# LayoutLLM-T2I/LayoutLLM-T2I

Measured on AMD Instinct MI355X. Metric: 512x512 50-step images/sec (PLMS, CFG 7.5, layout-conditioned GLIGEN UNet), higher is better.
Workload: dtype fp16 (fp32 accumulate); 1 GPU; configs[1]: 512x512, 50 PLMS steps, batch=4/GPU, 8 grounding boxes/image, fp16; survey_config=2, unet_forwards_per_image=102, parallelism=replicas x1, one weight broadcast, no per-step collectives

## Files before the change

layoutllm_t2i_amd/csrc/gemm_conv.hip:

```cpp
#include <atomic>
#include <cstring>
#include "common.h"
#include "gligen_hip.h"
#include "gemm_shared.h"
#include "opts.h"

namespace {

#define g_opt_ksplit gl_opt(13)
#define g_opt_geglu32 gl_opt(8)
#define g_opt_big gl_opt(7)
#define g_opt_small gl_opt(4)
#define g_opt_splitk_tiles gl_opt(5)
#define g_opt_splitk_tiles_conv gl_opt(GL_OPT_SPLITK_TILES_CONV)
#define g_opt_splitk_nk gl_opt(6)
#define g_opt_skinny gl_opt(24)
#define g_opt_order gl_opt(23)
#define g_opt_tile gl_opt(2)
#define g_opt_g8 gl_opt(30)
#define g_opt_g8_tiles gl_opt(31)
#define g_opt_g8_tapmajor gl_opt(33)
#define g_opt_g8_minkt gl_opt(34)
std::atomic<uint64_t> g8_launches{0};
#define g_opt_g8_shortk gl_opt(37)
#define g_opt_g8_bm128 gl_opt(46)
#define g_opt_g8_minblk gl_opt(47)
#define g_opt_g8_s3 gl_opt(52)
#define g_opt_g8_minnk gl_opt(35)

template <int BM, int BN, int BKT, int NW = 4>
constexpr int lds_bytes() {
    constexpr int pipe = 2 * (BM + BN) * BKT * (int)sizeof(half_t);
    constexpr int epi = NW * 32 * 68 * (int)sizeof(float);
    return pipe > epi ? pipe : epi;
}

template <int BM, int BN, int BKT, int WK = 1>
constexpr int min_waves() {
    if (WK > 1) return 2;
    if (BKT != 32) return 1;
    if (BM * BN >= 256 * 128) return 2;
    if (BM * BN <= 128 * 128) return 4;
    return 3;
}

template <int BM, int BN, int WAVES_M, int WAVES_N, bool CONV, int BKT, int WK = 1>
__global__ __launch_bounds__(64 * WAVES_M * WAVES_N * WK, (min_waves<BM, BN, BKT, WK>())) void gemm_kernel(gl_gemm_args p, ConvGeom cg, int splitk, int kt_per_split, int order_m) {
    constexpr int NTHR = 64 * WAVES_M * WAVES_N * WK;
    constexpr int TM = BM / WAVES_M / 32;
    constexpr int TN = BN / WAVES_N / 32;
    constexpr int CPR = BKT / 8;
    constexpr int RPP = NTHR / CPR;
    constexpr int RPW = 64 / CPR;
    constexpr int APASS = (BM + RPP - 1) / RPP;
    constexpr int BPASS = (BN + RPP - 1) / RPP;
    constexpr int KSTEPS = BKT / 16;
    static_assert(WAVES_M * WAVES_N * WK == 4, "4 waves");
    static_assert(WK == 1 || (WK == 2 && TM == 2 && KSTEPS % 2 == 0), "K-split: two groups, two 32-row tiles per wave");
    static_assert(BM % RPW == 0 && BN % RPW == 0, "whole wave instructions");
    static_assert(BKT == 64 || BKT == 32, "BK");

    extern __shared__ __attribute__((aligned(16))) unsigned char smem[];
    half_t* As = reinterpret_cast<half_t*>(smem);
    half_t* Bs = As + 2 * BM * BKT;

    const int tid = threadIdx.x;
    const int lane = tid & 63;
    const int wave = tid >> 6;
    const int wk = wave / (WAVES_M * WAVES_N);
    const int wmn = wave - wk * (WAVES_M * WAVES_N);
    const int wm = wmn / WAVES_N;
    const int wn = wmn % WAVES_N;
    const int M = p.M, N = p.N, K = p.K;
    const int nt = (N + BN - 1) / BN;
    int tile;
    {
        const int nwg = gridDim.x;
        const int bid = blockIdx.x;
        const int q = nwg >> 3, r = nwg & 7;
        const int xcd = bid & 7, local = bid >> 3;
        tile = (xcd < r ? xcd * (q + 1) : r * (q + 1) + (xcd - r) * q) + local;
    }
    const int mt_ = (M + BM - 1) / BM;
    const int tm = order_m ? tile % mt_ : tile / nt;
    const int m0 = tm * BM;
    const int n0 = (order_m ? tile / mt_ : tile - tm * nt) * BN;
    const int kt_begin = blockIdx.z * kt_per_split;
    const int kt_end = min(K / BKT, kt_begin + kt_per_split);
    const int nkt = kt_end - kt_begin;

    const int srow = tid / CPR;
    const int skc = tid % CPR;
    auto swz = [](int r) -> int { return BKT == 64 ? ((r >> 1) & 7) : ((r >> 2) & 3); };

    const half_t* __restrict__ Ag = reinterpret_cast<const half_t*>(p.a);
    const half_t* __restrict__ A2g = reinterpret_cast<const half_t*>(p.a2);
    const half_t* __restrict__ Wg = reinterpret_cast<const half_t*>(p.w);
    const half_t* zsrc = reinterpret_cast<const half_t*>(g_zero16);

// ... 328 lines not shown
                    const int pc = (lane & 3) * 8;
                    const int m = mbase + r;
                    const int nx = nbase + pc;
                    if (m < M && nx < N) {
                        const float4 x0 = *reinterpret_cast<const float4*>(stage + r * EPS + pc);
                        const float4 x1 = *reinterpret_cast<const float4*>(stage + r * EPS + pc + 4);
                        const float4 g0 = *reinterpret_cast<const float4*>(stage + r * EPS + pc + 32);
                        const float4 g1 = *reinterpret_cast<const float4*>(stage + r * EPS + pc + 36);
                        float xv[8] = {x0.x, x0.y, x0.z, x0.w, x1.x, x1.y, x1.z, x1.w};
                        float gv[8] = {g0.x, g0.y, g0.z, g0.w, g1.x, g1.y, g1.z, g1.w};
                        half8_t o, lo8 = {};
#pragma unroll
                        for (int j = 0; j < 8; ++j) {
                            float a = xv[j], b = gv[j];
                            if (bias) { a += bias[nx + j]; b += bias[nx + 32 + j]; }
                            float y = a * gelu_erf_f(b);
                            if (p.out_mode == GL_OUT_F16_HILO) y = pin_value(y);
                            o[j] = (half_t)y;
                            if (p.out_mode == GL_OUT_F16_HILO) lo8[j] = (half_t)(y - (float)o[j]);
                        }
                        st16(outp + (size_t)m * p.ldc + (nbase >> 1) + pc, *reinterpret_cast<uint4*>(&o));
                        if (p.out_mode == GL_OUT_F16_HILO) st16(outp + (size_t)m * p.ldc + (N >> 1) + (nbase >> 1) + pc, *reinterpret_cast<uint4*>(&lo8));
                    }
                }
            } else {
                const int ncols = (np * 2 + 1 < TN) ? 64 : 32;
#pragma unroll
                for (int ps = 0; ps < 4; ++ps) {
                    const int r = ps * 8 + (lane >> 3);
                    const int c = (lane & 7) * 8;
                    const int m = mbase + r;
                    const int n = nbase + c;
                    if (c < ncols && m < M && n < N) {
                        const float4 a0 = *reinterpret_cast<const float4*>(stage + r * EPS + c);
                        const float4 a1 = *reinterpret_cast<const float4*>(stage + r * EPS + c + 4);
                        float v[8] = {a0.x, a0.y, a0.z, a0.w, a1.x, a1.y, a1.z, a1.w};
                        finish8(p, gate, m, n, v);
                    }
                }
            }
        }
    }
}

__global__ __launch_bounds__(256) void splitk_reduce_kernel(gl_gemm_args p, int splitk) {
    const int M = p.M, N = p.N;
    const int nq = N / 8;
    const size_t total = (size_t)M * nq;
    const float* ws = reinterpret_cast<const float*>(p.workspace);
    float gate = 1.0f;
    if (p.epi == GL_EPI_GATE_RES) gate = p.gate[0];
    const size_t zstride = (size_t)M * N;
    for (unsigned idx = blockIdx.x * 256u + threadIdx.x; idx < (unsigned)total; idx += gridDim.x * 256u) {
        const int m = (int)(idx / (unsigned)nq);
        const int n = (int)(idx - (unsigned)m * (unsigned)nq) * 8;
        const float* src = ws + (size_t)m * N + n;
        float4 a = *reinterpret_cast<const float4*>(src);
        float4 c = *reinterpret_cast<const float4*>(src + 4);
        int z = 1;
        for (; z + 1 < splitk; z += 2) {
            const float4 b0 = *reinterpret_cast<const float4*>(src + (size_t)z * zstride);
            const float4 d0 = *reinterpret_cast<const float4*>(src + (size_t)z * zstride + 4);
            const float4 b1 = *reinterpret_cast<const float4*>(src + (size_t)(z + 1) * zstride);
            const float4 d1 = *reinterpret_cast<const float4*>(src + (size_t)(z + 1) * zstride + 4);
            a.x += b0.x; a.y += b0.y; a.z += b0.z; a.w += b0.w;
            c.x += d0.x; c.y += d0.y; c.z += d0.z; c.w += d0.w;
            a.x += b1.x; a.y += b1.y; a.z += b1.z; a.w += b1.w;
            c.x += d1.x; c.y += d1.y; c.z += d1.z; c.w += d1.w;
        }
        for (; z < splitk; ++z) {
            const float4 b = *reinterpret_cast<const float4*>(src + (size_t)z * zstride);
            const float4 d = *reinterpret_cast<const float4*>(src + (size_t)z * zstride + 4);
            a.x += b.x; a.y += b.y; a.z += b.z; a.w += b.w;
            c.x += d.x; c.y += d.y; c.z += d.z; c.w += d.w;
        }
        float v[8] = {a.x, a.y, a.z, a.w, c.x, c.y, c.z, c.w};
        finish8(p, gate, m, n, v);
    }
}

constexpr int SK_BATCH = 20;
constexpr int SK_RS = 36;

__global__ __launch_bounds__(256) void gemm_skinny_kernel(gl_gemm_args p) {
    __shared__ __attribute__((aligned(16))) float part[4][32 * SK_RS];
    const int lane = threadIdx.x & 63, wave = threadIdx.x >> 6;
    const int n0 = blockIdx.x * 32, m0 = blockIdx.y * 32;
    const int M = p.M, K = p.K;
    const int steps = K / 64;
    const int kw = wave * steps * 16;
    int mr = m0 + (lane & 31);
    if (mr >= M) mr = M - 1;
    const half_t* ap = reinterpret_cast<const half_t*>(p.a) + (size_t)mr * p.lda + kw + 8 * (lane >> 5);
    const half_t* wp = reinterpret_cast<const half_t*>(p.w) + (size_t)(n0 + (lane & 31)) * p.ldw + (p.kwrap != 0 && kw >= p.kwrap ? kw - p.kwrap : kw) +
                       8 * (lane >> 5);
    f32x16 acc;
#pragma unroll
    for (int j = 0; j < 16; ++j) acc[j] = 0.0f;
    for (int s0 = 0; s0 < steps; s0 += SK_BATCH) {
        uint4 af[SK_BATCH], wf[SK_BATCH];
#pragma unroll
        for (int j = 0; j < SK_BATCH; ++j)
            if (s0 + j < steps) {
                af[j] = ld16(ap + (s0 + j) * 16);
                wf[j] = ld16(wp + (s0 + j) * 16);
            }
#pragma unroll
        for (int j = 0; j < SK_BATCH; ++j)
            if (s0 + j < steps)
                acc = __builtin_amdgcn_mfma_f32_32x32x16_f16(*reinterpret_cast<half8_t*>(&wf[j]), *reinterpret_cast<half8_t*>(&af[j]), acc, 0, 0, 0);
    }
    float* mine = part[wave] + (lane & 31) * SK_RS + 4 * (lane >> 5);
#pragma unroll
    for (int rg = 0; rg < 4; ++rg)
        *reinterpret_cast<float4*>(mine + 8 * rg) = make_float4(acc[rg * 4], acc[rg * 4 + 1], acc[rg * 4 + 2], acc[rg * 4 + 3]);
    __syncthreads();
    if (threadIdx.x < 128) {
        const int r = threadIdx.x >> 2, c = (threadIdx.x & 3) * 8;
        const int m = m0 + r;
        if (m < M) {
            float v[8];
#pragma unroll
            for (int j = 0; j < 8; ++j) v[j] = part[0][r * SK_RS + c + j];
#pragma unroll
            for (int w = 1; w < 4; ++w)
#pragma unroll
                for (int j = 0; j < 8; ++j) v[j] += part[w][r * SK_RS + c + j];
            float gate = 1.0f;
            if (p.epi == GL_EPI_GATE_RES) gate = p.gate[0];
            finish8(p, gate, m, n0 + c, v);
        }
    }
}

inline bool skinny_ok(const gl_gemm_args& g) {
    if (!g_opt_skinny || g.M > 1024 || (g.N % 32) != 0 || g.epi == GL_EPI_GEGLU || g.vt != nullptr || g.a2 != nullptr) return false;
    if (g.kwrap != 0 && g.K != 2 * g.kwrap) return false;
    if (g.out_mode == GL_OUT_F32_NCHW || (g.lda % 8) != 0) return false;
    if (g.K > 4096 && g.workspace != nullptr) return false;
    const long tiles = (long)gl_cdiv(g.M, 32) * (g.N / 32);
    return tiles * 64L * g.K * 2L <= (long)g_opt_skinny << 20;
}

inline int choose_splitk(const gl_gemm_args& g, int tiles, bool conv) {
    const int nk = g.K / 64;
    if (!g.workspace || g.epi == GL_EPI_GEGLU || g.out_mode == GL_OUT_F32_NCHW || g.vt != nullptr) return 1;
    if (tiles >= (conv ? g_opt_splitk_tiles_conv : g_opt_splitk_tiles) || nk < g_opt_splitk_nk) return 1;
    int s = (480 + tiles - 1) / tiles;
    if (s > nk / 8) s = nk / 8;
    if (s > 16) s = 16;
    while (s > 1 && (int64_t)s * g.M * g.N * 4 > g.workspace_bytes) --s;
    return s < 2 ? 1 : s;
}

template <int BM, int BN, int WM, int WN, bool CONV, int BKT, int WK = 1>
int launch(const gl_gemm_args& g, const ConvGeom& cg, hipStream_t st) {
    if (g.a2 != nullptr && (g.ksplit % BKT) != 0) return GL_ERR_BAD_ARG;
    if (g.vt != nullptr && ((g.vt_col0 % BN) % 64) != 0) return GL_ERR_UNSUPPORTED;
    const int mt = gl_cdiv(g.M, BM), nt = gl_cdiv(g.N, BN);
    const int nk = g.K / BKT;
    int splitk = choose_splitk(g, mt * nt, CONV);
    int kper = gl_cdiv(nk, splitk);
    const int zs = gl_cdiv(nk, kper);
    dim3 grid(mt * nt, 1, zs);
    constexpr int lds = lds_bytes<BM, BN, BKT, WM * WN * WK>();
    const int order_m = g_opt_order == 1 ? ((CONV ? 9L : 1L) * g.N > (long)g.M) : (g_opt_order == 2);
    gemm_kernel<BM, BN, WM, WN, CONV, BKT, WK><<<grid, dim3(64 * WM * WN * WK), lds, st>>>(g, cg, zs, kper, order_m);
    GL_CHECK_LAUNCH();
    if (zs > 1) {
        const size_t total = (size_t)g.M * (g.N / 8);
        int nblk = (int)((total + 255) / 256);
        if (nblk > 2048) nblk = 2048;
        splitk_reduce_kernel<<<dim3(nblk), dim3(256), 0, st>>>(g, zs);
        GL_CHECK_LAUNCH();
    }
    return 0;
}

template <bool CONV, int BKT>
int dispatch_shape(const gl_gemm_args& g, const ConvGeom& cg, hipStream_t st) {
    const bool geglu = (g.epi == GL_EPI_GEGLU);
    const bool rowmajor = (g.out_mode != GL_OUT_F32_NCHW);
    int shape = 0;
    if (g.N < 256 && (g.N % 128) != 0) shape = 2;
    else if (!geglu && (g.N % 160) == 0 && ((g.N % 128) != 0 || CONV || g_opt_tile == 2)) shape = 1;
    if (g_opt_tile == 1 && g.N >= 256) shape = 0;
    if (g_opt_small && !CONV && g.K <= 1280 && shape != 2 && (g.N % 128) == 0) {
        const long t128 = (long)gl_cdiv(g.M, 128) * gl_cdiv(g.N, shape == 1 ? 160 : 128);
        if (t128 < g_opt_small) shape = 3;
    }
    if constexpr (BKT == 64) {
        if (g_opt_ksplit && rowmajor && (shape == 0 || shape == 1)) {
            const int nk = g.K / 64;
            bool use = (g_opt_ksplit == 2);
            if (g_opt_ksplit == 1 || g_opt_ksplit == 3 || g_opt_ksplit == 4) use = CONV ? (shape == 1 && nk >= 20) : (nk >= 16);
            if (g_opt_ksplit == 3 && !CONV) use = false;
            if (g_opt_ksplit == 4 && CONV) use = false;
            if (use) {
                if (shape == 1) return launch<128, 160, 2, 1, CONV, 64, 2>(g, cg, st);
                return launch<128, 128, 2, 1, CONV, 64, 2>(g, cg, st);
            }
        }
        if (g_opt_big && shape != 2 && shape != 3 && g.M >= 256 && !(shape == 1 && g.vt != nullptr)) {
            const int bn = (shape == 1) ? 160 : 128;
            const long t256 = (long)gl_cdiv(g.M, 256) * gl_cdiv(g.N, bn);
            if (t256 >= g_opt_big) {
                if (shape == 1) return launch<256, 160, 4, 1, CONV, 32>(g, cg, st);
                return launch<256, 128, 4, 1, CONV, 32>(g, cg, st);
            }
        }
        if constexpr (!CONV) {
            if (shape == 3 && (g_opt_ksplit == 2 || ((g_opt_ksplit == 1 || g_opt_ksplit == 4 || g_opt_ksplit == 5) && g.K >= 1024)))
                return launch<64, 128, 1, 2, false, 64, 2>(g, cg, st);
        }
        if (shape == 3) return launch<64, 128, 2, 2, CONV, 64>(g, cg, st);
        if (shape == 1) return launch<128, 160, 4, 1, CONV, 64>(g, cg, st);
        if (shape == 0) return launch<128, 128, 2, 2, CONV, 64>(g, cg, st);
        return launch<256, 64, 4, 1, CONV, 64>(g, cg, st);
    } else {
        static_assert(!CONV, "BK 32 dispatch is for plain GEMMs");
        if (shape == 3) return launch<64, 128, 2, 2, false, 32>(g, cg, st);
        return launch<128, 128, 2, 2, false, 32>(g, cg, st);
    }
}

template <bool CONV>
int dispatch(const gl_gemm_args& g, const ConvGeom& cg, hipStream_t st) {
    if (g.M <= 0 || g.N <= 0 || g.K <= 0 || (g.K % 64) != 0) return GL_ERR_BAD_ARG;
    if (g.out_mode < 0 || g.out_mode > GL_OUT_F16_HILO) return GL_ERR_BAD_ARG;
    if (g.out_mode == GL_OUT_F16_HILO && g.ldc < (g.epi == GL_EPI_GEGLU ? g.N : 2 * g.N)) return GL_ERR_BAD_ARG;
    if ((g.vt != nullptr && (g.out_mode == GL_OUT_F16_HILO) != (g.vt_lo != nullptr)) || (g.vt == nullptr && g.vt_lo != nullptr)) return GL_ERR_BAD_ARG;
    if (g.out_mode != GL_OUT_F32_NCHW && ((g.N % 8) != 0 || (g.ldc % 8) != 0)) return GL_ERR_BAD_ARG;
    if (g.out_mode == GL_OUT_F32_ROWMAJOR && g.out2 != nullptr && (g.ldc2 % 8) != 0) return GL_ERR_BAD_ARG;
    if (g.out_mode == GL_OUT_F32_ROWMAJOR && g.epi == GL_EPI_GEGLU) return GL_ERR_UNSUPPORTED;
    if (g.res != nullptr && (g.ldres % 8) != 0) return GL_ERR_BAD_ARG;
    if (g.rowbias != nullptr && (g.ld_rowbias % 8) != 0) return GL_ERR_BAD_ARG;
    if (g.epi == GL_EPI_GEGLU && (g.N % 64) != 0) return GL_ERR_BAD_ARG;
    if (g.a2 != nullptr && (g.ksplit % 64) != 0) return GL_ERR_BAD_ARG;
    if ((g.epi == GL_EPI_RES || g.epi == GL_EPI_GATE_RES) && g.res == nullptr) return GL_ERR_BAD_ARG;
    if (g.epi == GL_EPI_GATE_RES && g.gate == nullptr) return GL_ERR_BAD_ARG;
    if (g.epi == GL_EPI_ROWBIAS && (g.rowbias == nullptr || g.rows_per_sample <= 0)) return GL_ERR_BAD_ARG;
    if (g.vt != nullptr && (g.epi != GL_EPI_BIAS || (g.out_mode != GL_OUT_F16_ROWMAJOR && g.out_mode != GL_OUT_F16_HILO) || (g.vt_col0 % 64) != 0 || g.vt_col0 <= 0 ||
                            g.vt_col0 >= g.N || g.vt_rows <= 0 || g.vt_d <= 0 || ((g.N - g.vt_col0) % g.vt_d) != 0 || (g.vt_ld % 8) != 0 ||
                            g.vt_ld < g.vt_rows || g.vt_H * g.vt_d != g.N - g.vt_col0))
        return GL_ERR_BAD_ARG;
    if constexpr (!CONV) {
        if (g.vt_lo == nullptr && skinny_ok(g)) {
            gemm_skinny_kernel<<<dim3(g.N / 32, gl_cdiv(g.M, 32)), dim3(256), 0, st>>>(g);
            GL_CHECK_LAUNCH();
            return 0;
        }
    }
    const bool need8 = g.vt_lo != nullptr;
    if (need8) {
        int bn_ = 0;
        if (!g_opt_g8 || !gl8_supported(g, CONV, &bn_)) return GL_ERR_UNSUPPORTED;
    }
    const bool upf = CONV && cg.ups == 2;
    auto mtiles = [&](const int bm_) { return upf ? 4 * gl_cdiv(g.M / 4, bm_) : gl_cdiv(g.M, bm_); };
    if (g_opt_g8 || upf) {
        int bn = 0;
        if (gl8_supported(g, CONV, &bn, upf)) {
            const int nk = g.K / 64;
            auto plan_split = [&](const int tiles_) {
                int sk = 1;
                if (tiles_ < g_opt_g8_tiles && g.workspace && g.epi != GL_EPI_GEGLU && g.vt == nullptr) {
                    sk = 256 / tiles_;
                    if (sk > nk / g_opt_g8_minkt) sk = nk / g_opt_g8_minkt;
                    while (sk > 1 && (int64_t)sk * g.M * g.N * 4 > g.workspace_bytes) --sk;
                    if (sk < 1) sk = 1;
                }
                return sk;
            };
            int bm = 256;
            int tiles = mtiles(256) * gl_cdiv(g.N, bn);
            int splitk = plan_split(tiles);
            if (tiles * 2 <= 256 && g.epi != GL_EPI_GEGLU && g.vt == nullptr) {
                const bool want = CONV ? ((g_opt_g8_bm128 & 4) || ((g_opt_g8_bm128 & 1) && nk / splitk <= 16)) : ((g_opt_g8_bm128 & 2) != 0);
                if (want) {
                    bm = 128;
                    tiles = mtiles(128) * gl_cdiv(g.N, bn);
                    splitk = plan_split(tiles);
                }
            }
            if (!CONV && (g_opt_g8_bm128 & 8) && bm == 256 && splitk == 1 && tiles > 256 && g.epi != GL_EPI_GEGLU) {
                const int t128 = gl_cdiv(g.M, 128) * gl_cdiv(g.N, bn);
                auto fills = [](const int b) { return b * 5 >= ((b + 255) / 256) * 256 * 4; };
                if (!fills(tiles) && fills(t128) && t128 <= 2048) {
                    bm = 128;
                    tiles = t128;
                }
            }
            if (!CONV && splitk > 1 && nk / splitk < 20) splitk = nk / 20 > 0 ? nk / 20 : 1;
            bool enough = tiles * splitk >= (CONV ? g_opt_g8_tiles : (g_opt_g8_minblk < g_opt_g8_tiles ? g_opt_g8_minblk : g_opt_g8_tiles)) && nk >= g_opt_g8_minnk;
            if (!CONV && enough) {
                const int blocks = tiles * splitk;
                const bool full_rounds = g_opt_g8_shortk && blocks * 5 >= ((blocks + 255) / 256) * 256 * 4;
                enough = nk >= 16 || blocks <= 256 || (g.epi == GL_EPI_GEGLU && (nk >= 10 || full_rounds)) || (full_rounds && blocks <= 2048);
            }
            if (g_opt_g8 == 2 || enough || need8 || upf) {
                const bool s3 = g_opt_g8_s3 != 0 && g.kwrap != 0 && g.K == 3 * g.kwrap &&
                                (CONV ? cg.cwrap != 0 : (g.a2 == g.a && g.lda2 == g.lda && g.ksplit == 2 * g.kwrap));
                const int nks = s3 ? g.kwrap / 32 : nk;
                const int kper = gl_cdiv(nks, splitk);
                const int zs = gl_cdiv(nks, kper);
                const int order_m = g_opt_order == 1 ? ((CONV ? 9L : 1L) * g.N > (long)g.M) : (g_opt_order == 2);
                const int e = gl8_launch(g, cg, CONV, bm, bn, zs, kper, order_m | (CONV && g_opt_g8_tapmajor ? 2 : 0), st, s3);
                if (e) return e;
                if (!upf) g8_launches.fetch_add(1, std::memory_order_relaxed);
                if (zs > 1) {
                    const size_t total = (size_t)g.M * (g.N / 8);
                    int nblk = (int)((total + 255) / 256);
                    if (nblk > 2048) nblk = 2048;
                    splitk_reduce_kernel<<<dim3(nblk), dim3(256), 0, st>>>(g, zs);
                    GL_CHECK_LAUNCH();
                }
                return 0;
            }
        }
    }
    if (upf) return GL_ERR_UNSUPPORTED;
    if constexpr (!CONV) {
        if (g_opt_geglu32 && g.epi == GL_EPI_GEGLU && g.K <= 640 && g.a2 == nullptr) return dispatch_shape<false, 32>(g, cg, st);
    }
    return dispatch_shape<CONV, 64>(g, cg, st);
}

}

extern "C" int gl_gemm(const gl_gemm_args* a, void* stream) {
    if (!a || !a->a || !a->w || !a->out) return GL_ERR_BAD_ARG;
    ConvGeom cg{};
    gl_gemm_args g = *a;
    if (g.kwrap != 0 && ((g.kwrap % 64) != 0 || g.kwrap >= g.K || g.K > 3 * g.kwrap)) return GL_ERR_BAD_ARG;
    if (g.ldw == 0) g.ldw = g.kwrap != 0 ? g.kwrap : g.K;
    if (g.ldw < (g.kwrap != 0 ? (g.K > 2 * g.kwrap ? 2 * g.kwrap : g.kwrap) : g.K) || (g.ldw % 8) != 0) return GL_ERR_BAD_ARG;
    return dispatch<false>(g, cg, (hipStream_t)stream);
}

namespace {
int conv3x3_entry(const gl_conv_args* a, int shift, void* stream) {
    if (!a || !a->in || !a->g.w || !a->g.out) return GL_ERR_BAD_ARG;
    if ((a->Cin % 64) != 0) return GL_ERR_BAD_ARG;
    if (a->stride != 1 && a->stride != 2) return GL_ERR_BAD_ARG;
    if (a->upsample2x < 0 || a->upsample2x > 2) return GL_ERR_BAD_ARG;
    if (a->upsample2x && (a->stride != 1 || a->Hout != 2 * a->Hin || a->Wout != 2 * a->Win)) return GL_ERR_BAD_ARG;
    const bool upf = a->upsample2x == 2;
    if (upf && (shift != 0 || a->in_split != 0 || a->w_split != 0 || a->g.out_mode == GL_OUT_F32_NCHW || a->g.out_mode == GL_OUT_F16_HILO ||
                a->g.epi == GL_EPI_GEGLU || a->g.vt != nullptr || a->g.vt_lo != nullptr))
        return GL_ERR_BAD_ARG;
    if (a->B >= 2048 || a->Hout >= 1024 || a->Wout >= 1024) return GL_ERR_BAD_ARG;
    if (a->in_split != 0 && a->in_split != 2 && a->in_split != 3) return GL_ERR_BAD_ARG;
    if (a->in_split == 3 && !a->w_split) return GL_ERR_BAD_ARG;
    gl_gemm_args g = a->g;
    g.a = a->in;
    g.a2 = nullptr;
    g.M = a->B * a->Hout * a->Wout;
    g.K = 9 * a->Cin * (a->in_split ? a->in_split : 1);
    g.ldw = 9 * a->Cin * (a->w_split ? 2 : 1);
    g.kwrap = a->in_split ? 9 * a->Cin : 0;
    if (upf) g.K = g.ldw = 4 * a->Cin;
    ConvGeom cg{reinterpret_cast<const half_t*>(a->in), a->B, a->Hin, a->Win, a->Cin * (a->in_split ? 2 : 1), a->Hout, a->Wout, a->stride,
                a->upsample2x, nullptr, a->in_split == 3 ? 2 * (a->Cin >> 6) : 0, shift};
    return dispatch<true>(g, cg, (hipStream_t)stream);
}
}

extern "C" int gl_conv3x3(const gl_conv_args* a, void* stream) { return conv3x3_entry(a, 0, stream); }

extern "C" int gl_conv3x3_pad01(const gl_conv_args* a, void* stream) {
    if (!a || a->stride != 2 || a->upsample2x != 0 || a->in_split != 0) return GL_ERR_BAD_ARG;
    if (a->Hout != a->Hin / 2 || a->Wout != a->Win / 2 || a->Hout <= 0 || a->Wout <= 0) return GL_ERR_BAD_ARG;
    return conv3x3_entry(a, 1, stream);
}

template <int BM, int BN, int WM, int WN, bool CONV, int BKT, int WK = 1>
int set_lds_attr() {
    hipError_t e = hipFuncSetAttribute((const void*)gemm_kernel<BM, BN, WM, WN, CONV, BKT, WK>,
                                       hipFuncAttributeMaxDynamicSharedMemorySize, lds_bytes<BM, BN, BKT, WM * WN * WK>());
    return e == hipSuccess ? 0 : (int)e;
}
template <int BM, int BN, int WM, int WN, int BKT, int WK = 1>
int set_lds_attr2() {
    int e = set_lds_attr<BM, BN, WM, WN, false, BKT, WK>();
    return e ? e : set_lds_attr<BM, BN, WM, WN, true, BKT, WK>();
}

extern "C" int gl_init_gemm(void) {
    int e;
    if ((e = set_lds_attr2<64, 128, 2, 2, 64>())) return e;
    if ((e = set_lds_attr2<128, 128, 2, 2, 64>())) return e;
    if ((e = set_lds_attr2<128, 160, 4, 1, 64>())) return e;
    if ((e = set_lds_attr2<256, 64, 4, 1, 64>())) return e;
    if ((e = set_lds_attr2<128, 160, 2, 1, 64, 2>())) return e;
    if ((e = set_lds_attr2<128, 128, 2, 1, 64, 2>())) return e;
    if ((e = set_lds_attr<64, 128, 1, 2, false, 64, 2>())) return e;
    if ((e = set_lds_attr2<256, 160, 4, 1, 32>())) return e;
    if ((e = set_lds_attr2<256, 128, 4, 1, 32>())) return e;
    if ((e = set_lds_attr<64, 128, 2, 2, false, 32>())) return e;
    if ((e = set_lds_attr<128, 128, 2, 2, false, 32>())) return e;
    if ((e = gl8_init())) return e;
    return 0;
}

int gl_attn_read_launch_counts(void* dst, int64_t bytes);

extern "C" int gl_debug_read(int what, void* dst, int64_t bytes) {
    if (what == 8) return gl8_read_stamps(dst, bytes);
    if (what == 10) return gl_attn_read_launch_counts(dst, bytes);
    if (what == 9 || what == 11 || what == 12) {
        if (!dst || bytes < (int64_t)sizeof(uint64_t)) return GL_ERR_BAD_ARG;
        const uint64_t n = what == 9 ? g8_launches.load(std::memory_order_relaxed) : (what == 11 ? gl8_kxr_launch_count() : gl8_upf_launch_count());
        memcpy(dst, &n, sizeof n);
        return 0;
    }
    return GL_ERR_BAD_ARG;
}
```

layoutllm_t2i_amd/csrc/misc.hip:

```cpp
#include "common.h"
#include "gligen_hip.h"
#include "opts.h"

namespace {

template <typename OT>
__global__ __launch_bounds__(256) void posnet_input_kernel(const float* __restrict__ boxes, const float* __restrict__ masks,
                                                           const float* __restrict__ emb, const float* __restrict__ null_pos,
                                                           const float* __restrict__ null_xyxy, int in_dim, int num_freqs,
                                                           OT* __restrict__ out) {
    const int row = blockIdx.x;
    const float m = masks[row];
    const int pos_dim = num_freqs * 8;
    OT* o = out + (size_t)row * (in_dim + pos_dim);
    for (int c = threadIdx.x; c < in_dim; c += 256) {
        const float v = emb[(size_t)row * in_dim + c] * m + (1.0f - m) * null_pos[c];
        o[c] = (OT)v;
    }
    for (int c = threadIdx.x; c < pos_dim; c += 256) {
        const int j = c / 8;
        const int r = c - j * 8;
        const int coord = r & 3;
        const float freq = powf(100.0f, (float)j / (float)num_freqs);
        const float arg = freq * boxes[(size_t)row * 4 + coord];
// ... 506 lines not shown

extern "C" int gl_pack_latent(const float* x, int32_t B, int32_t C, int32_t hw, int32_t Cpad, int32_t reps, int32_t split, void* out,
                              void* stream) {
    if (!x || !out || B <= 0 || C <= 0 || hw <= 0 || Cpad < (split ? 3 * C : C) || reps <= 0) return GL_ERR_BAD_ARG;
    pack_latent_kernel<<<dim3(ew_blocks((size_t)reps * B * hw * Cpad)), dim3(256), 0, (hipStream_t)stream>>>(
        x, B, C, hw, Cpad, reps, split, reinterpret_cast<half_t*>(out));
    GL_CHECK_LAUNCH();
    return 0;
}

extern "C" int gl_pack_latent_extra(const float* x, const float* extra, int32_t B, int32_t Bs, int32_t C, int32_t Ce, int32_t hw, int32_t Cpad,
                                    int32_t reps, int32_t split, void* out, void* stream) {
    if (!x || !extra || !out || B <= 0 || C <= 0 || Ce <= 0 || hw <= 0 || reps <= 0 || (Bs != 1 && Bs != B)) return GL_ERR_BAD_ARG;
    if (Cpad < (split ? 3 : 1) * (C + Ce)) return GL_ERR_BAD_ARG;
    pack_latent_extra_kernel<<<dim3(ew_blocks((size_t)reps * B * hw * Cpad)), dim3(256), 0, (hipStream_t)stream>>>(
        x, extra, B, Bs, C, Ce, hw, Cpad, reps, split, reinterpret_cast<half_t*>(out));
    GL_CHECK_LAUNCH();
    return 0;
}

extern "C" int gl_latent_blend(float* x, const float* x0, const float* noise, const float* mask, float a, float s, int32_t B, int32_t C,
                               int32_t hw, int32_t x0_batch, int32_t mask_batch, void* stream) {
    if (!x || !x0 || !noise || !mask || B <= 0 || C <= 0 || hw <= 0) return GL_ERR_BAD_ARG;
    if ((x0_batch != 1 && x0_batch != B) || (mask_batch != 1 && mask_batch != B)) return GL_ERR_BAD_ARG;
    const size_t n = (size_t)B * C * hw;
    const bool vec = (hw % 4) == 0 && ((reinterpret_cast<uintptr_t>(x) | reinterpret_cast<uintptr_t>(x0) | reinterpret_cast<uintptr_t>(noise) |
                                        reinterpret_cast<uintptr_t>(mask)) % 16) == 0;
    if (vec)
        latent_blend_kernel<4><<<dim3(ew_blocks(n / 4)), dim3(256), 0, (hipStream_t)stream>>>(x, x0, noise, mask, a, s, B, C, hw, x0_batch, mask_batch);
    else
        latent_blend_kernel<1><<<dim3(ew_blocks(n)), dim3(256), 0, (hipStream_t)stream>>>(x, x0, noise, mask, a, s, B, C, hw, x0_batch, mask_batch);
    GL_CHECK_LAUNCH();
    return 0;
}

extern "C" int gl_vae_posterior(const float* h, const float* w, const float* bias, const float* noise, float scale, int32_t B, int32_t Cin,
                                int32_t E, int32_t hw, float* z, float* mean, void* stream) {
    if (!h || !w || !bias || !noise || !z || B <= 0 || Cin <= 0 || E <= 0 || hw <= 0) return GL_ERR_BAD_ARG;
    vae_posterior_kernel<<<dim3(ew_blocks((size_t)B * hw)), dim3(256), 0, (hipStream_t)stream>>>(h, w, bias, noise, scale, B, Cin, E, hw, z, mean);
    GL_CHECK_LAUNCH();
    return 0;
}

extern "C" int gl_softmax_rows(void* x, int32_t rows, int32_t n, int32_t ld, float scale, void* stream) {
    if (!x || rows <= 0 || n <= 0 || (n % 8) || (ld % 8)) return GL_ERR_BAD_ARG;
    softmax_rows_kernel<<<dim3(rows), dim3(256), 0, (hipStream_t)stream>>>(reinterpret_cast<half_t*>(x), n, ld, scale);
    GL_CHECK_LAUNCH();
    return 0;
}

extern "C" int gl_latent_affine_pack(const float* z, const float* w, const float* bias, float pre, int32_t B, int32_t C,
                                     int32_t hw, int32_t Cpad, void* out, void* stream) {
    if (!z || !w || !bias || !out || B <= 0 || C <= 0 || hw <= 0 || Cpad < C) return GL_ERR_BAD_ARG;
    latent_affine_pack_kernel<<<dim3(ew_blocks((size_t)B * hw * Cpad)), dim3(256), 0, (hipStream_t)stream>>>(
        z, w, bias, pre, B, C, hw, Cpad, reinterpret_cast<half_t*>(out));
    GL_CHECK_LAUNCH();
    return 0;
}

extern "C" int gl_init_gemm(void);
extern "C" int gl_init_ff(void);
extern "C" int gl_init_attn(void);
static gl_opts make_default_opts() {
    gl_opts o{};
    o.v[2] = 0;    o.v[3] = 0;    o.v[4] = 400;  o.v[5] = 300;  o.v[GL_OPT_SPLITK_TILES_CONV] = 450;
    o.v[6] = 16;   o.v[7] = 300;  o.v[8] = 1;    o.v[10] = -1;  o.v[13] = 3;
    o.v[16] = 16;  o.v[17] = 1;   o.v[20] = 0;   o.v[21] = 1;   o.v[23] = 1;
    o.v[24] = 64;  o.v[25] = 1;   o.v[27] = 1;   o.v[29] = 1;   o.v[30] = 1;
    o.v[31] = 200; o.v[32] = 0;   o.v[33] = 0;   o.v[34] = 11;  o.v[35] = 5;
    o.v[37] = 1;
    o.v[41] = 1;
    o.v[42] = 1;
    o.v[43] = 1;
    o.v[38] = 1;
    o.v[44] = 1;
    o.v[45] = 1024;
    o.v[46] = 11;
    o.v[47] = 100;
    o.v[50] = 0;
    o.v[51] = 1;
    o.v[52] = 1;
    o.v[55] = 2;
    o.v[54] = 2;
    return o;
}
gl_opts g_gl_opts = make_default_opts();
thread_local const gl_opts* tl_gl_opts = nullptr;
int g_gl_option_epoch = 0;

bool gl_opts_put(gl_opts& t, int key, int value) {
    switch (key) {
        case 2: case 3: case 4: case 6: case 7: case 8: case 10: case 13: case 17: case 20: case 21: case 23: case 24: case 25:
        case 27: case 29: case 30: case 31: case 32: case 33: case 35: case 37: case 38: case 41: case 42: case 43: case 44: case 45: case 46: case 47: case 50: case 51: case 52: case 53: case 54: case 55:
            t.v[key] = value;
            return true;
        case 5:
            t.v[5] = value < 0 ? 300 : value;
            t.v[GL_OPT_SPLITK_TILES_CONV] = value < 0 ? 450 : value;
            return true;
        case 16: t.v[16] = value > 0 ? value : 16; return true;
        case 34: t.v[34] = value < 1 ? 1 : value; return true;
        default: return false;
    }
}

extern "C" int gl_get_option(int key) {
    if (key < 0 || key >= GL_OPT_MAX) return GL_ERR_BAD_ARG;
    return g_gl_opts.v[key];
}

extern "C" int gl_set_option(int key, int value) {
    if (key < 0 || key >= GL_OPT_MAX || !gl_opts_put(g_gl_opts, key, value)) return GL_ERR_BAD_ARG;
    ++g_gl_option_epoch;
    return 0;
}

extern "C" int gl_abi_version(void) { return GL_ABI_VERSION; }
extern "C" int gl_sizeof_gemm_args(void) { return (int)sizeof(gl_gemm_args); }
extern "C" int gl_sizeof_conv_args(void) { return (int)sizeof(gl_conv_args); }
extern "C" int gl_sizeof_attn_args(void) { return (int)sizeof(gl_attn_args); }
extern "C" int gl_sizeof_gn_args(void) { return (int)sizeof(gl_gn_args); }
extern "C" int gl_init(void) {
    int e = gl_init_gemm();
    if (!e) e = gl_init_ff();
    return e ? e : gl_init_attn();
}
```

layoutllm_t2i_amd/csrc/opts.h:

```cpp
#pragma once
#include <cstdint>

constexpr int GL_OPT_MAX = 56;
constexpr int GL_OPT_SPLITK_TILES_CONV = 40;

struct gl_opts {
    int v[GL_OPT_MAX];
};

struct gl_opt_overrides {
    uint64_t mask = 0;
    int v[GL_OPT_MAX] = {};
    int epoch = 0;
};

extern gl_opts g_gl_opts;
extern int g_gl_option_epoch;
extern thread_local const gl_opts* tl_gl_opts;

static inline int gl_opt(int key) {
    const gl_opts* o = tl_gl_opts;
    return (o ? o : &g_gl_opts)->v[key];
}

bool gl_opts_put(gl_opts& t, int key, int value);

struct gl_opts_scope {
    gl_opts eff;
    const gl_opts* prev;
    explicit gl_opts_scope(const gl_opt_overrides& o) : prev(tl_gl_opts) {
        eff = g_gl_opts;
        for (int k = 0; k < GL_OPT_MAX; ++k)
            if ((o.mask >> k) & 1u) gl_opts_put(eff, k, o.v[k]);
        tl_gl_opts = &eff;
    }
    ~gl_opts_scope() { tl_gl_opts = prev; }
    gl_opts_scope(const gl_opts_scope&) = delete;
    gl_opts_scope& operator=(const gl_opts_scope&) = delete;
};
```

layoutllm_t2i_amd/ops.py:

```python
from __future__ import annotations

import ctypes as C
from typing import Optional

import torch

from . import _lib
from ._lib import (EPI_BIAS, EPI_GATE_RES, EPI_GEGLU, EPI_RES, EPI_ROWBIAS, EPI_SILU, OUT_F16_HILO, OUT_F16_ROWMAJOR, OUT_F32_NCHW,
                   OUT_F32_ROWMAJOR, AttnArgs, ConvArgs, GemmArgs, GnArgs, check)

F16 = torch.float16
F32 = torch.float32


_DEV = None


def _stream() -> int:
    dev = _DEV if _DEV is not None else torch.cuda.current_device()
    if dev != torch.cuda.current_device():
        raise _lib.HipLibraryError(f"tensors live on cuda:{dev} but cuda:{torch.cuda.current_device()} is current: wrap the "
                                   "call in torch.cuda.device(...) (kernels launch on the current device)")
    _lib.init_device(dev)
    return torch.cuda.current_stream(dev).cuda_stream
# ... 543 lines not shown
    return out


def vae_posterior(h: torch.Tensor, w: torch.Tensor, bias: torch.Tensor, noise: torch.Tensor, scale: float, z: torch.Tensor,
                  mean: Optional[torch.Tensor] = None) -> torch.Tensor:
    for t, n in ((h, "h"), (w, "w"), (bias, "bias"), (noise, "noise"), (z, "z")):
        _req(t, F32, n, 4)
    B, Cin, hh, ww = h.shape
    E = w.shape[0] // 2
    if w.shape != (2 * E, Cin) or tuple(z.shape) != (B, E, hh, ww) or noise.shape != z.shape:
        raise ValueError("vae_posterior: w [2E, Cin], noise / z [B, E, h, w]")
    if mean is not None:
        _req(mean, F32, "mean", 4)
    check(_lib.lib().gl_vae_posterior(h.data_ptr(), w.data_ptr(), bias.data_ptr(), noise.data_ptr(), float(scale), B, Cin, E, hh * ww,
                                      z.data_ptr(), _ptr(mean), _stream()), "gl_vae_posterior")
    return z


def latent_blend(x: torch.Tensor, x0: torch.Tensor, noise: torch.Tensor, mask: torch.Tensor, a: float, s: float) -> torch.Tensor:
    for t, n in ((x, "x"), (x0, "x0"), (noise, "noise"), (mask, "mask")):
        _req(t, F32, n, 4)
    B, Cc, hh, ww = x.shape
    if x0.shape[1:] != x.shape[1:] or noise.shape != x0.shape or x0.shape[0] not in (1, B) or \
            tuple(mask.shape[1:]) != (1, hh, ww) or mask.shape[0] not in (1, B):
        raise ValueError("latent_blend: x0 / noise [1|B, C, h, w], mask [1|B, 1, h, w]")
    check(_lib.lib().gl_latent_blend(x.data_ptr(), x0.data_ptr(), noise.data_ptr(), mask.data_ptr(), float(a), float(s), B, Cc, hh * ww,
                                     x0.shape[0], mask.shape[0], _stream()), "gl_latent_blend")
    return x


def softmax_rows(x: torch.Tensor, scale: float = 1.0) -> torch.Tensor:
    _req(x, F16, "x")
    rows, n, ld = _rows(x, "x")
    check(_lib.lib().gl_softmax_rows(x.data_ptr(), rows, n, ld, scale, _stream()), "gl_softmax_rows")
    return x


def latent_affine_pack(z: torch.Tensor, w: torch.Tensor, bias: torch.Tensor, pre: float, Cpad: int, out: torch.Tensor):
    for t, n in ((z, "z"), (w, "w"), (bias, "bias")):
        _req(t, F32, n, 4)
    _req(out, F16, "out")
    B, Cc, h, ww = z.shape
    check(_lib.lib().gl_latent_affine_pack(z.data_ptr(), w.data_ptr(), bias.data_ptr(), pre, B, Cc, h * ww, Cpad,
                                           out.data_ptr(), _stream()), "gl_latent_affine_pack")
    return out


def set_option(key: int, value: int) -> None:
    check(_lib.lib().gl_set_option(key, value), "gl_set_option")


def gemm8_launch_count() -> int:
    import ctypes
    n = ctypes.c_uint64(0)
    check(_lib.lib().gl_debug_read(9, ctypes.byref(n), 8), "gl_debug_read")
    return int(n.value)


def kxreuse_launch_count() -> int:
    import ctypes
    n = ctypes.c_uint64(0)
    check(_lib.lib().gl_debug_read(11, ctypes.byref(n), 8), "gl_debug_read")
    return int(n.value)


def upfold_launch_count() -> int:
    import ctypes
    n = ctypes.c_uint64(0)
    check(_lib.lib().gl_debug_read(12, ctypes.byref(n), 8), "gl_debug_read")
    return int(n.value)


ATTN_FORMS = ("split_pipe", "split_8w", "split_4w_dbuf", "split_4w_single", "f16_8w_pre0", "f16_8w_pre1", "f16_8w_pre2", "f16_4w_pre0",
              "f16_4w_pre1", "f16_4w_pre2")


def attention_launch_counts() -> dict:
    import ctypes
    n = (ctypes.c_uint64 * len(ATTN_FORMS))()
    check(_lib.lib().gl_debug_read(10, ctypes.byref(n), ctypes.sizeof(n)), "gl_debug_read")
    return {k: int(v) for k, v in zip(ATTN_FORMS, n)}


def clip_patchify(pixel_values: torch.Tensor, patch: int, Kpad: int, out: torch.Tensor) -> torch.Tensor:
    _req(pixel_values, F32, "pixel_values")
    _req(out, F16, "out")
    B, c3, S, S2 = pixel_values.shape
    if c3 != 3 or S != S2 or not pixel_values.is_contiguous():
        raise ValueError("pixel_values must be a contiguous [B, 3, S, S] tensor")
    check(_lib.lib().gl_clip_patchify(pixel_values.data_ptr(), B, S, patch, Kpad, out.data_ptr(), _stream()), "gl_clip_patchify")
    return out


def clip_assemble(patch_emb: torch.Tensor, class_emb: torch.Tensor, pos_emb: torch.Tensor, B: int, T: int, x: torch.Tensor,
                  ln_gamma: Optional[torch.Tensor] = None, ln_beta: Optional[torch.Tensor] = None, eps: float = 1e-5) -> torch.Tensor:
    _req(patch_emb, F16, "patch_emb")
    for t, n in ((class_emb, "class_emb"), (pos_emb, "pos_emb"), (x, "x")):
        _req(t, F32, n)
    C_ = x.shape[-1]
    check(_lib.lib().gl_clip_assemble(patch_emb.data_ptr(), _rows(patch_emb, "patch_emb")[2], class_emb.data_ptr(), pos_emb.data_ptr(), B, T, C_,
                                      _ptr(ln_gamma), _ptr(ln_beta), eps, x.data_ptr(), _stream()), "gl_clip_assemble")
    return x


def clip_embed_tokens(ids: torch.Tensor, tok_emb: torch.Tensor, pos_emb: torch.Tensor, x: torch.Tensor) -> torch.Tensor:
    _req(ids, torch.int32, "ids", 4)
    for t, n in ((tok_emb, "tok_emb"), (pos_emb, "pos_emb"), (x, "x")):
        _req(t, F32, n)
    B, T = ids.shape
    check(_lib.lib().gl_clip_embed_tokens(ids.data_ptr(), tok_emb.data_ptr(), pos_emb.data_ptr(), B, T, x.shape[-1], tok_emb.shape[0],
                                          x.data_ptr(), _stream()), "gl_clip_embed_tokens")
    return x


def clip_gather_rows(x: torch.Tensor, rows: torch.Tensor, out: torch.Tensor) -> torch.Tensor:
    _req(x, F32, "x")
    _req(rows, torch.int32, "rows", 4)
    _req(out, F32, "out")
    check(_lib.lib().gl_clip_gather_rows(x.data_ptr(), _rows(x, "x")[2], rows.data_ptr(), rows.numel(), x.shape[-1], out.data_ptr(), _stream()),
          "gl_clip_gather_rows")
    return out


def attention_small(q: torch.Tensor, k: torch.Tensor, v: torch.Tensor, ld: int, B: int, T: int, H: int, d: int, scale: float,
                    causal: bool, out: torch.Tensor) -> torch.Tensor:
    for t, n in ((q, "q"), (k, "k"), (v, "v")):
        _req(t, F16, n, 2)
    _req(out, F16, "out", 2)
    check(_lib.lib().gl_attention_small(q.data_ptr(), k.data_ptr(), v.data_ptr(), ld, B, T, H, d, scale, int(causal), out.data_ptr(),
                                        _rows(out, "out")[2], _stream()), "gl_attention_small")
    return out


def image_to_u8(img: torch.Tensor, out: torch.Tensor) -> torch.Tensor:
    _req(img, F32, "img")
    B, c3, H, W = img.shape
    if c3 != 3 or not img.is_contiguous() or out.dtype != torch.uint8 or tuple(out.shape) != (B, H, W, 3) or not out.is_contiguous():
        raise ValueError("img must be contiguous fp32 [B, 3, H, W] and out contiguous uint8 [B, H, W, 3]")
    check(_lib.lib().gl_image_to_u8(img.data_ptr(), B, H, W, out.data_ptr(), _stream()), "gl_image_to_u8")
    return out


def _req_tables(bounds: torch.Tensor, coeffs: torch.Tensor, n_out: int, ksize: int) -> None:
    if bounds.dtype != torch.int32 or coeffs.dtype != torch.int32 or not bounds.is_cuda or not coeffs.is_cuda:
        raise ValueError("bounds / coeffs must be int32 tensors on the GPU")
    if tuple(bounds.shape) != (n_out, 2) or tuple(coeffs.shape) != (n_out, ksize) or not bounds.is_contiguous() or not coeffs.is_contiguous():
        raise ValueError("bounds must be [n_out, 2] and coeffs [n_out, ksize], contiguous")


def resample_h_u8(x: torch.Tensor, bounds: torch.Tensor, coeffs: torch.Tensor, ksize: int, out: torch.Tensor) -> torch.Tensor:
    if x.dtype != torch.uint8 or out.dtype != torch.uint8 or not x.is_cuda or not out.is_cuda or not x.is_contiguous() or not out.is_contiguous():
        raise ValueError("x / out must be contiguous uint8 tensors on the GPU")
    B, H, W, _ = x.shape
    Wout = out.shape[2]
    if tuple(out.shape) != (B, H, Wout, 3):
        raise ValueError("out must be [B, H, Wout, 3]")
    _req_tables(bounds, coeffs, Wout, ksize)
    check(_lib.lib().gl_resample_h_u8(x.data_ptr(), B, H, W, bounds.data_ptr(), coeffs.data_ptr(), ksize, Wout, out.data_ptr(), _stream()),
          "gl_resample_h_u8")
    return out


def resample_v_norm(x: torch.Tensor, bounds: torch.Tensor, coeffs: torch.Tensor, ksize: int, Hout: int, top: int, left: int, crop_h: int,
                    crop_w: int, mean, std, out: Optional[torch.Tensor], out_u8: Optional[torch.Tensor] = None):
    import ctypes

# ... 167 lines not shown
```

Baseline: 5.198 images/s.

## Generalize skinny GEMM to multi-tile, variable waves, and fused GEGLU epilogue

Templates the skinny MFMA GEMM on wave count, M-tiles per block and a GEGLU mode, so small-M GEMMs (M<=64) can cover two 32-row tiles per block and split K over 4, 8 or 16 waves. The GEGLU variant computes both the value and gate halves and applies the gelu gate in the epilogue, letting GEGLU feed-forward layers with few rows use the skinny path instead of the general tiled kernel. By default (mode 2) it is used only for GEGLU shapes with 320<=K<=1280 and M>32. It adds a staged cross-wave LDS reduction and per-form launch counters, which cost extra syncs and atomics per launch.

Result: no change. 5.224 images/s (median of 6 runs) (+0.5%).

```diff
diff --git a/layoutllm_t2i_amd/csrc/gemm_conv.hip b/layoutllm_t2i_amd/csrc/gemm_conv.hip
--- a/layoutllm_t2i_amd/csrc/gemm_conv.hip
+++ b/layoutllm_t2i_amd/csrc/gemm_conv.hip
@@ -15,6 +15,7 @@
 #define g_opt_splitk_tiles_conv gl_opt(GL_OPT_SPLITK_TILES_CONV)
 #define g_opt_splitk_nk gl_opt(6)
 #define g_opt_skinny gl_opt(24)
+#define g_opt_skinny2 gl_opt(56)
 #define g_opt_order gl_opt(23)
 #define g_opt_tile gl_opt(2)
 #define g_opt_g8 gl_opt(30)
@@ -509,53 +510,111 @@
 constexpr int SK_BATCH = 20;
 constexpr int SK_RS = 36;
 
-__global__ __launch_bounds__(256) void gemm_skinny_kernel(gl_gemm_args p) {
-    __shared__ __attribute__((aligned(16))) float part[4][32 * SK_RS];
+template <int NW, int MT, bool GEGLU>
+constexpr int sk_batch() {
+    if (NW == 4) return MT == 1 && !GEGLU ? SK_BATCH : 10;
+    if (NW == 8) return 10;
+    return GEGLU ? 2 : (MT == 1 ? 10 : 5);
+}
+template <int MT, bool GEGLU>
+constexpr int sk_round() { return MT * (GEGLU ? 2 : 1) == 4 ? 2 : 4; }
+
+template <int NW, int MT, bool GEGLU>
+__global__ __launch_bounds__(64 * NW) void gemm_skinny_kernel(gl_gemm_args p) {
+    constexpr int WT = GEGLU ? 2 : 1;
+    constexpr int SB = sk_batch<NW, MT, GEGLU>();
+    constexpr int RW = sk_round<MT, GEGLU>();
+    static_assert(SB >= 1 && NW % RW == 0, "skinny form");
+    __shared__ __attribute__((aligned(16))) float part[RW][MT * WT][32 * SK_RS];
     const int lane = threadIdx.x & 63, wave = threadIdx.x >> 6;
-    const int n0 = blockIdx.x * 32, m0 = blockIdx.y * 32;
+    const int n0 = blockIdx.x * 32, m0 = blockIdx.y * (32 * MT);
     const int M = p.M, K = p.K;
-    const int steps = K / 64;
+    const int steps = K / (16 * NW);
     const int kw = wave * steps * 16;
-    int mr = m0 + (lane & 31);
-    if (mr >= M) mr = M - 1;
-    const half_t* ap = reinterpret_cast<const half_t*>(p.a) + (size_t)mr * p.lda + kw + 8 * (lane >> 5);
-    const half_t* wp = reinterpret_cast<const half_t*>(p.w) + (size_t)(n0 + (lane & 31)) * p.ldw + (p.kwrap != 0 && kw >= p.kwrap ? kw - p.kwrap : kw) +
+    const half_t* ap[MT];
+#pragma unroll
+    for (int t = 0; t < MT; ++t) {
+        int mr = m0 + 32 * t + (lane & 31);
+        if (mr >= M) mr = M - 1;
+        ap[t] = reinterpret_cast<const half_t*>(p.a) + (size_t)mr * p.lda + kw + 8 * (lane >> 5);
+    }
+    const half_t* wp = reinterpret_cast<const half_t*>(p.w) + (size_t)(n0 * WT + (lane & 31)) * p.ldw + (p.kwrap != 0 && kw >= p.kwrap ? kw - p.kwrap : kw) +
                        8 * (lane >> 5);
-    f32x16 acc;
-#pragma unroll
-    for (int j = 0; j < 16; ++j) acc[j] = 0.0f;
-    for (int s0 = 0; s0 < steps; s0 += SK_BATCH) {
-        uint4 af[SK_BATCH], wf[SK_BATCH];
-#pragma unroll
-        for (int j = 0; j < SK_BATCH; ++j)
+    f32x16 acc[MT][WT];
+#pragma unroll
+    for (int t = 0; t < MT; ++t)
+#pragma unroll
+        for (int u = 0; u < WT; ++u)
+#pragma unroll
+            for (int j = 0; j < 16; ++j) acc[t][u][j] = 0.0f;
+    for (int s0 = 0; s0 < steps; s0 += SB) {
+        uint4 af[MT][SB], wf[WT][SB];
+#pragma unroll
+        for (int j = 0; j < SB; ++j)
             if (s0 + j < steps) {
-                af[j] = ld16(ap + (s0 + j) * 16);
-                wf[j] = ld16(wp + (s0 + j) * 16);
-            }
-#pragma unroll
-        for (int j = 0; j < SK_BATCH; ++j)
-            if (s0 + j < steps)
-                acc = __builtin_amdgcn_mfma_f32_32x32x16_f16(*reinterpret_cast<half8_t*>(&wf[j]), *reinterpret_cast<half8_t*>(&af[j]), acc, 0, 0, 0);
-    }
-    float* mine = part[wave] + (lane & 31) * SK_RS + 4 * (lane >> 5);
-#pragma unroll
-    for (int rg = 0; rg < 4; ++rg)
-        *reinterpret_cast<float4*>(mine + 8 * rg) = make_float4(acc[rg * 4], acc[rg * 4 + 1], acc[rg * 4 + 2], acc[rg * 4 + 3]);
-    __syncthreads();
-    if (threadIdx.x < 128) {
-        const int r = threadIdx.x >> 2, c = (threadIdx.x & 3) * 8;
-        const int m = m0 + r;
-        if (m < M) {
-            float v[8];
-#pragma unroll
-            for (int j = 0; j < 8; ++j) v[j] = part[0][r * SK_RS + c + j];
-#pragma unroll
-            for (int w = 1; w < 4; ++w)
-#pragma unroll
-                for (int j = 0; j < 8; ++j) v[j] += part[w][r * SK_RS + c + j];
+#pragma unroll
+                for (int t = 0; t < MT; ++t) af[t][j] = ld16(ap[t] + (s0 + j) * 16);
+#pragma unroll
+                for (int u = 0; u < WT; ++u) wf[u][j] = ld16(wp + (size_t)(32 * u) * p.ldw + (s0 + j) * 16);
+            }
+#pragma unroll
+        for (int j = 0; j < SB; ++j)
+            if (s0 + j < steps) {
+#pragma unroll
+                for (int t = 0; t < MT; ++t)
+#pragma unroll
+                    for (int u = 0; u < WT; ++u)
+                        acc[t][u] = __builtin_amdgcn_mfma_f32_32x32x16_f16(*reinterpret_cast<half8_t*>(&wf[u][j]), *reinterpret_cast<half8_t*>(&af[t][j]),
+                                                                           acc[t][u], 0, 0, 0);
+            }
+    }
+    const int rt = (threadIdx.x >> 7) & (MT - 1), r = (threadIdx.x >> 2) & 31, c = (threadIdx.x & 3) * 8;
+    float v[WT][8];
+#pragma unroll
+    for (int w0 = 0; w0 < NW; w0 += RW) {
+        if (w0 != 0) __syncthreads();
+        if (wave >= w0 && wave < w0 + RW) {
+#pragma unroll
+            for (int t = 0; t < MT; ++t)
+#pragma unroll
+                for (int u = 0; u < WT; ++u) {
+                    float* mine = part[wave - w0][t * WT + u] + (lane & 31) * SK_RS + 4 * (lane >> 5);
+#pragma unroll
+                    for (int rg = 0; rg < 4; ++rg)
+                        *reinterpret_cast<float4*>(mine + 8 * rg) = make_float4(acc[t][u][rg * 4], acc[t][u][rg * 4 + 1], acc[t][u][rg * 4 + 2], acc[t][u][rg * 4 + 3]);
+                }
+        }
+        __syncthreads();
+        if (threadIdx.x < 128 * MT) {
+#pragma unroll
+            for (int u = 0; u < WT; ++u) {
+                if (w0 == 0) {
+#pragma unroll
+                    for (int j = 0; j < 8; ++j) v[u][j] = part[0][rt * WT + u][r * SK_RS + c + j];
+                }
+#pragma unroll
+                for (int w = (w0 == 0 ? 1 : 0); w < RW; ++w)
+#pragma unroll
+                    for (int j = 0; j < 8; ++j) v[u][j] += part[w][rt * WT + u][r * SK_RS + c + j];
+            }
+        }
+    }
+    const int m = m0 + 32 * rt + r;
+    if (threadIdx.x < 128 * MT && m < M) {
+        if constexpr (GEGLU) {
+            const int nx = 2 * n0 + c;
+            half8_t o;
+#pragma unroll
+            for (int j = 0; j < 8; ++j) {
+                float a = v[0][j], b = v[WT - 1][j];
+                if (p.bias) { a += p.bias[nx + j]; b += p.bias[nx + 32 + j]; }
+                o[j] = (half_t)(a * gelu_erf_f(b));
+            }
+            st16(reinterpret_cast<half_t*>(p.out) + (size_t)m * p.ldc + n0 + c, *reinterpret_cast<uint4*>(&o));
+        } else {
             float gate = 1.0f;
             if (p.epi == GL_EPI_GATE_RES) gate = p.gate[0];
-            finish8(p, gate, m, n0 + c, v);
+            finish8(p, gate, m, n0 + c, v[0]);
         }
     }
 }
@@ -567,6 +626,58 @@
     if (g.K > 4096 && g.workspace != nullptr) return false;
     const long tiles = (long)gl_cdiv(g.M, 32) * (g.N / 32);
     return tiles * 64L * g.K * 2L <= (long)g_opt_skinny << 20;
+}
+
+struct SkinnyPlan {
+    int nw, mt, geglu;
+};
+
+constexpr int SK_FORMS = 12;
+std::atomic<uint64_t> skinny_launches[SK_FORMS];
+
+inline bool skinny_plan_measured(const gl_gemm_args& g, SkinnyPlan& pl) {
+    if (!pl.geglu || g.M <= 32 || g.K < 320 || g.K > 1280) return false;
+    pl.nw = (g.K >= 640 && (g.K % 128) == 0) ? 8 : 4;
+    pl.mt = 2 * (g.N / 64) > 256 ? 2 : 1;
+    return true;
+}
+
+inline bool skinny_plan(const gl_gemm_args& g, SkinnyPlan& pl) {
+    const int mode = g_opt_skinny2 & 15, force = (g_opt_skinny2 >> 4) & 31, force_mt = (g_opt_skinny2 >> 9) & 3;
+    if (!mode || !g_opt_skinny || g.M > 64 || g.vt != nullptr || g.a2 != nullptr || g.kwrap != 0) return false;
+    if (g.out_mode == GL_OUT_F32_NCHW || (g.lda % 8) != 0) return false;
+    pl.geglu = g.epi == GL_EPI_GEGLU;
+    if (pl.geglu ? ((g.N % 64) != 0 || g.out_mode != GL_OUT_F16_ROWMAJOR) : (g.N % 32) != 0) return false;
+    pl.mt = g.M > 32 ? 2 : 1;
+    pl.nw = g.K <= 640 ? 4 : (g.K <= 1280 ? 8 : 16);
+    if (mode == 2 && !force && !force_mt && !skinny_plan_measured(g, pl)) return false;
+    if (force == 4 || force == 8 || force == 16) pl.nw = force;
+    if (force_mt == 1 || force_mt == 2) pl.mt = force_mt;
+    if (g.K > 5120 || (g.K % (16 * pl.nw)) != 0) return false;
+    const long tiles = (long)gl_cdiv(g.M, 32 * pl.mt) * (g.N / (pl.geglu ? 64 : 32));
+    if (tiles * (32L * pl.mt + (pl.geglu ? 64L : 32L)) * g.K * 2L > (long)g_opt_skinny << 20) return false;
+    return true;
+}
+
+template <int NW, int MT, bool GEGLU>
+void skinny_launch_form(const gl_gemm_args& g, hipStream_t st) {
+    gemm_skinny_kernel<NW, MT, GEGLU><<<dim3(g.N / (GEGLU ? 64 : 32), gl_cdiv(g.M, 32 * MT)), dim3(64 * NW), 0, st>>>(g);
+    skinny_launches[((NW == 4 ? 0 : NW == 8 ? 1 : 2) * 2 + (MT - 1)) * 2 + (GEGLU ? 1 : 0)].fetch_add(1, std::memory_order_relaxed);
+}
+template <int NW>
+void skinny_launch_nw(const gl_gemm_args& g, const SkinnyPlan& pl, hipStream_t st) {
+    if (pl.mt == 2) {
+        if (pl.geglu) skinny_launch_form<NW, 2, true>(g, st);
+        else skinny_launch_form<NW, 2, false>(g, st);
+    } else {
+        if (pl.geglu) skinny_launch_form<NW, 1, true>(g, st);
+        else skinny_launch_form<NW, 1, false>(g, st);
+    }
+}
+inline void skinny_launch(const gl_gemm_args& g, const SkinnyPlan& pl, hipStream_t st) {
+    if (pl.nw == 4) skinny_launch_nw<4>(g, pl, st);
+    else if (pl.nw == 8) skinny_launch_nw<8>(g, pl, st);
+    else skinny_launch_nw<16>(g, pl, st);
 }
 
 inline int choose_splitk(const gl_gemm_args& g, int tiles, bool conv) {
@@ -672,8 +783,14 @@
                             g.vt_ld < g.vt_rows || g.vt_H * g.vt_d != g.N - g.vt_col0))
         return GL_ERR_BAD_ARG;
     if constexpr (!CONV) {
+        SkinnyPlan pl;
+        if (g.vt_lo == nullptr && skinny_plan(g, pl)) {
+            skinny_launch(g, pl, st);
+            GL_CHECK_LAUNCH();
+            return 0;
+        }
         if (g.vt_lo == nullptr && skinny_ok(g)) {
-            gemm_skinny_kernel<<<dim3(g.N / 32, gl_cdiv(g.M, 32)), dim3(256), 0, st>>>(g);
+            skinny_launch_form<4, 1, false>(g, st);
             GL_CHECK_LAUNCH();
             return 0;
         }
@@ -835,6 +952,13 @@
 extern "C" int gl_debug_read(int what, void* dst, int64_t bytes) {
     if (what == 8) return gl8_read_stamps(dst, bytes);
     if (what == 10) return gl_attn_read_launch_counts(dst, bytes);
+    if (what == 13) {
+        if (!dst || bytes < (int64_t)(SK_FORMS * sizeof(uint64_t))) return GL_ERR_BAD_ARG;
+        uint64_t n[SK_FORMS];
+        for (int i = 0; i < SK_FORMS; ++i) n[i] = skinny_launches[i].load(std::memory_order_relaxed);
+        memcpy(dst, n, sizeof n);
+        return 0;
+    }
     if (what == 9 || what == 11 || what == 12) {
         if (!dst || bytes < (int64_t)sizeof(uint64_t)) return GL_ERR_BAD_ARG;
         const uint64_t n = what == 9 ? g8_launches.load(std::memory_order_relaxed) : (what == 11 ? gl8_kxr_launch_count() : gl8_upf_launch_count());
diff --git a/layoutllm_t2i_amd/csrc/misc.hip b/layoutllm_t2i_amd/csrc/misc.hip
--- a/layoutllm_t2i_amd/csrc/misc.hip
+++ b/layoutllm_t2i_amd/csrc/misc.hip
@@ -612,6 +612,7 @@
     o.v[52] = 1;
     o.v[55] = 2;
     o.v[54] = 2;
+    o.v[56] = 2;
     return o;
 }
 gl_opts g_gl_opts = make_default_opts();
@@ -621,7 +622,7 @@
 bool gl_opts_put(gl_opts& t, int key, int value) {
     switch (key) {
         case 2: case 3: case 4: case 6: case 7: case 8: case 10: case 13: case 17: case 20: case 21: case 23: case 24: case 25:
-        case 27: case 29: case 30: case 31: case 32: case 33: case 35: case 37: case 38: case 41: case 42: case 43: case 44: case 45: case 46: case 47: case 50: case 51: case 52: case 53: case 54: case 55:
+        case 27: case 29: case 30: case 31: case 32: case 33: case 35: case 37: case 38: case 41: case 42: case 43: case 44: case 45: case 46: case 47: case 50: case 51: case 52: case 53: case 54: case 55: case 56:
             t.v[key] = value;
             return true;
         case 5:
diff --git a/layoutllm_t2i_amd/csrc/opts.h b/layoutllm_t2i_amd/csrc/opts.h
--- a/layoutllm_t2i_amd/csrc/opts.h
+++ b/layoutllm_t2i_amd/csrc/opts.h
@@ -1,7 +1,7 @@
 #pragma once
 #include <cstdint>
 
-constexpr int GL_OPT_MAX = 56;
+constexpr int GL_OPT_MAX = 57;
 constexpr int GL_OPT_SPLITK_TILES_CONV = 40;
 
 struct gl_opts {
diff --git a/layoutllm_t2i_amd/ops.py b/layoutllm_t2i_amd/ops.py
--- a/layoutllm_t2i_amd/ops.py
+++ b/layoutllm_t2i_amd/ops.py
@@ -649,6 +649,16 @@
     return {k: int(v) for k, v in zip(ATTN_FORMS, n)}
 
 
+SKINNY_FORMS = tuple((nw, mt, geglu) for nw in (4, 8, 16) for mt in (1, 2) for geglu in (False, True))
+
+
+def skinny_launch_counts() -> dict:
+    import ctypes
+    n = (ctypes.c_uint64 * len(SKINNY_FORMS))()
+    check(_lib.lib().gl_debug_read(13, ctypes.byref(n), ctypes.sizeof(n)), "gl_debug_read")
+    return {k: int(v) for k, v in zip(SKINNY_FORMS, n)}
+
+
 def clip_patchify(pixel_values: torch.Tensor, patch: int, Kpad: int, out: torch.Tensor) -> torch.Tensor:
     _req(pixel_values, F32, "pixel_values")
     _req(out, F16, "out")
```
